# xiaomo9/FAC_fake

Measured on AMD Instinct MI355X. Metric: face-crops/sec at 224x224 bf16, CViT forward, 1/2/4/8 MI355X, higher is better.
Workload: dtype bf16; 1 GPU; config 2: CViT forward, B=256 crops per GPU per step, pos slot j mod 32; model=CViT(224,7,2,512,1024,6,8,2048), global_batch=256, seq_len=2, parallelism=frame-sharded x1, graph=False, stem_chunk=0, fused_stem224=True, pipelined=True

## Files before the change

fac_fake_amd/_lib.py:

```python
from __future__ import annotations

import ctypes
import os
from pathlib import Path

import torch

LIB_PATH = Path(os.environ.get("FAC_CVIT_LIB", Path(__file__).resolve().parent / "libfac_cvit.so"))

FAC_OK = 0
STATUS = {0: "FAC_OK", -1: "FAC_ERR_ARG", -2: "FAC_ERR_SHAPE", -3: "FAC_ERR_MISSING", -4: "FAC_ERR_HIP",
          -5: "FAC_ERR_NOT_LOADED", -6: "FAC_ERR_OOM"}
DTYPES = {"bf16": 0, "fp16": 1}

SIGNATURES = {
    "fac_create": (ctypes.c_int, [ctypes.c_int, ctypes.c_int, ctypes.POINTER(ctypes.c_void_p)]),
    "fac_load_weights": (ctypes.c_int, [ctypes.c_void_p, ctypes.c_void_p, ctypes.c_int]),
    "fac_reserve": (ctypes.c_int, [ctypes.c_void_p, ctypes.c_int]),
    "fac_workspace_bytes": (ctypes.c_int, [ctypes.c_void_p, ctypes.c_int, ctypes.POINTER(ctypes.c_size_t)]),
    "fac_forward_nchw_f32": (ctypes.c_int, [ctypes.c_void_p, ctypes.c_void_p, ctypes.c_int, ctypes.c_void_p,
                                            ctypes.c_void_p, ctypes.c_void_p, ctypes.c_void_p]),
    "fac_forward_nhwc_u8": (ctypes.c_int, [ctypes.c_void_p, ctypes.c_void_p, ctypes.c_int, ctypes.c_void_p,
                                           ctypes.c_void_p, ctypes.c_void_p, ctypes.c_void_p]),
    "fac_forward_nhwc_u8_pipelined": (ctypes.c_int, [ctypes.c_void_p, ctypes.c_void_p, ctypes.c_int,
# ... 66 lines not shown
                                             ctypes.c_int, ctypes.c_void_p]),
    "fac_s3d_base0_u8": (ctypes.c_int, [ctypes.c_void_p, ctypes.c_void_p, ctypes.c_void_p, ctypes.c_int, ctypes.c_int,
                                        ctypes.c_int, ctypes.c_void_p]),
    "fac_conv_nd_dual": (ctypes.c_int, [ctypes.c_void_p, ctypes.c_void_p, ctypes.c_void_p]),
    "fac_sep_tiny": (ctypes.c_int, [ctypes.c_void_p, ctypes.c_void_p, ctypes.c_void_p]),
    "fac_sep_mid": (ctypes.c_int, [ctypes.c_void_p, ctypes.c_void_p, ctypes.c_void_p]),
    "fac_bottleneck_pw2": (ctypes.c_int, [ctypes.c_void_p, ctypes.c_void_p, ctypes.c_void_p]),
    "fac_conv_weight_layout": (ctypes.c_int, [ctypes.c_int, ctypes.c_int, ctypes.c_int, ctypes.c_int, ctypes.c_int,
                                              ctypes.POINTER(ctypes.c_int), ctypes.POINTER(ctypes.c_int)]),
    "fac_pool_nd": (ctypes.c_int, [ctypes.c_void_p, ctypes.c_void_p]),
    "fac_pack_input": (ctypes.c_int, [ctypes.c_int, ctypes.c_void_p, ctypes.c_int, ctypes.c_int, ctypes.c_int,
                                      ctypes.c_float, ctypes.c_void_p, ctypes.c_void_p, ctypes.c_void_p, ctypes.c_int,
                                      ctypes.c_void_p]),
    "fac_pack_input_s2d": (ctypes.c_int, [ctypes.c_int, ctypes.c_void_p, ctypes.c_int, ctypes.c_int, ctypes.c_int,
                                          ctypes.c_int, ctypes.c_int, ctypes.c_int, ctypes.c_int, ctypes.c_float,
                                          ctypes.c_void_p, ctypes.c_void_p, ctypes.c_void_p, ctypes.c_void_p]),
    "fac_kan_linear": (ctypes.c_int, [ctypes.c_void_p, ctypes.c_int, ctypes.c_int, ctypes.c_int, ctypes.c_void_p,
                                      ctypes.c_int, ctypes.c_void_p, ctypes.c_void_p, ctypes.c_void_p,
                                      ctypes.c_void_p]),
    "fac_kan_scratch_bytes": (ctypes.c_size_t, [ctypes.c_int, ctypes.c_int, ctypes.c_int]),
    "fac_sigmoid": (ctypes.c_int, [ctypes.c_void_p, ctypes.c_void_p, ctypes.c_int, ctypes.c_void_p]),
    "fac_conv_nd_split": (ctypes.c_int, [ctypes.c_void_p, ctypes.c_void_p, ctypes.c_int, ctypes.c_int, ctypes.c_void_p,
                                          ctypes.c_int, ctypes.c_int, ctypes.c_void_p]),
    "fac_conv_nd_route": (ctypes.c_char_p, [ctypes.c_void_p, ctypes.c_int, ctypes.c_int,
                                            ctypes.POINTER(ctypes.c_int)]),
    "fac_conv_nd_dual_route": (ctypes.c_char_p, [ctypes.c_void_p, ctypes.c_void_p, ctypes.POINTER(ctypes.c_int)]),
    "fac_pool_nd_route": (ctypes.c_char_p, [ctypes.c_void_p, ctypes.POINTER(ctypes.c_int)]),
    "fac_conv3x3_packed_elems": (ctypes.c_size_t, [ctypes.c_int, ctypes.c_int, ctypes.c_int]),
    "fac_conv3x3_pack": (ctypes.c_int, [ctypes.c_int, ctypes.c_int, ctypes.c_int, ctypes.c_int, ctypes.c_void_p,
                                        ctypes.c_void_p]),
    "fac_conv3x3": (ctypes.c_int, [ctypes.c_int, ctypes.c_void_p, ctypes.c_void_p, ctypes.c_void_p, ctypes.c_void_p,
                                   ctypes.c_int, ctypes.c_int, ctypes.c_int, ctypes.c_int, ctypes.c_int, ctypes.c_int,
                                   ctypes.c_void_p, ctypes.c_void_p]),
    "fac_conv3x3_res_packed_elems": (ctypes.c_size_t, [ctypes.c_int, ctypes.c_int]),
    "fac_conv3x3_res_pack": (ctypes.c_int, [ctypes.c_int, ctypes.c_int, ctypes.c_int, ctypes.c_void_p,
                                            ctypes.c_void_p]),
    "fac_conv3x3_res": (ctypes.c_int, [ctypes.c_int, ctypes.c_void_p, ctypes.c_void_p, ctypes.c_void_p,
                                       ctypes.c_void_p, ctypes.c_void_p, ctypes.c_int, ctypes.c_int, ctypes.c_int,
                                       ctypes.c_void_p]),
    "fac_avgpool_f32": (ctypes.c_int, [ctypes.c_int, ctypes.c_void_p, ctypes.c_int, ctypes.c_int, ctypes.c_int,
                                       ctypes.c_void_p, ctypes.c_void_p]),
    "fac_stem224_pack_conv1": (ctypes.c_int, [ctypes.c_int, ctypes.c_void_p, ctypes.c_void_p]),
    "fac_stem224": (ctypes.c_int, [ctypes.c_int, ctypes.c_int, ctypes.c_void_p, ctypes.c_void_p, ctypes.c_void_p,
                                   ctypes.c_void_p, ctypes.c_void_p, ctypes.c_void_p, ctypes.c_void_p, ctypes.c_void_p,
                                   ctypes.c_int, ctypes.c_void_p]),
    "fac_ggca": (ctypes.c_int, [ctypes.c_int, ctypes.c_void_p, ctypes.c_int, ctypes.c_int, ctypes.c_int, ctypes.c_int,
                                ctypes.c_int, ctypes.c_void_p, ctypes.c_void_p, ctypes.c_void_p, ctypes.c_void_p,
                                ctypes.c_void_p, ctypes.c_void_p, ctypes.c_void_p]),
    "fac_ggca_apply_route": (ctypes.c_int, [ctypes.c_int, ctypes.c_int, ctypes.c_int, ctypes.c_int]),
    "fac_ggca_apply": (ctypes.c_int, [ctypes.c_int, ctypes.c_void_p, ctypes.c_int, ctypes.c_int, ctypes.c_int,
                                      ctypes.c_int, ctypes.c_int, ctypes.c_void_p, ctypes.c_void_p, ctypes.c_void_p,
                                      ctypes.c_void_p, ctypes.c_void_p, ctypes.c_int, ctypes.c_void_p,
                                      ctypes.c_void_p]),
    "fac_ggca_scale": (ctypes.c_int, [ctypes.c_int, ctypes.c_void_p, ctypes.c_int, ctypes.c_int, ctypes.c_int,
                                      ctypes.c_int, ctypes.c_int, ctypes.c_void_p, ctypes.c_void_p, ctypes.c_void_p,
                                      ctypes.c_void_p, ctypes.c_void_p, ctypes.c_void_p, ctypes.c_void_p]),
    "fac_idwconv": (ctypes.c_int, [ctypes.c_int, ctypes.c_void_p, ctypes.c_void_p, ctypes.c_int, ctypes.c_int,
                                   ctypes.c_int, ctypes.c_int, ctypes.c_void_p, ctypes.c_void_p, ctypes.c_void_p,
                                   ctypes.c_void_p, ctypes.c_void_p, ctypes.c_int, ctypes.c_void_p]),
    "fac_smfa_scratch_bytes": (ctypes.c_size_t, [ctypes.c_int, ctypes.c_int, ctypes.c_int, ctypes.c_int]),
    "fac_smfa_packed_bytes": (ctypes.c_size_t, [ctypes.c_int]),
    "fac_smfa_pack": (ctypes.c_int, [ctypes.c_int, ctypes.c_int] + [ctypes.c_void_p] * 12),
    "fac_smfa": (ctypes.c_int, [ctypes.c_int, ctypes.c_void_p, ctypes.c_int, ctypes.c_int, ctypes.c_int, ctypes.c_int,
                                ctypes.c_void_p, ctypes.c_int, ctypes.c_void_p, ctypes.c_void_p, ctypes.c_void_p,
                                ctypes.c_void_p]),
    "fac_bfm_packed_elems": (ctypes.c_size_t, [ctypes.c_int]),
# ... 97 lines not shown
```

fac_fake_amd/csrc/conv.hip:

```cpp
#include <cstdlib>
#include <type_traits>

#include "common.hpp"

namespace fac {

constexpr int CONV_CK = 32;

__device__ __forceinline__ void glds16(const void* gsrc, void* ldst) {
  __builtin_amdgcn_global_load_lds((const __attribute__((address_space(1))) void*)gsrc,
                                   (__attribute__((address_space(3))) void*)ldst, 16, 0, 0);
}

template <int TW>
constexpr int halo_rp() { return TW + 2 <= 24 ? 24 : 40; }

template <int TH, int TW, int BN>
constexpr int tile_res() {
  return TW == 16 ? (BN == 32 ? 224 : 112) : (TH == 8 ? 56 : (TH == 4 ? 28 : (TH == 14 ? 14 : 0)));
}

template <int TW>
__device__ __forceinline__ void box_pixel(int m, int& py, int& px) {
  constexpr int WW = TW / 2;
// ... 277 lines not shown
      if (c == 0) CONV_STAMP(2 + t);
#endif
    };
    step(std::integral_constant<int, 0>{});
    step(std::integral_constant<int, 1>{});
    step(std::integral_constant<int, 2>{});
    step(std::integral_constant<int, 3>{});
    step(std::integral_constant<int, 4>{});
    step(std::integral_constant<int, 5>{});
    step(std::integral_constant<int, 6>{});
    step(std::integral_constant<int, 7>{});
    step(std::integral_constant<int, 8>{});
  }
  asm volatile("s_waitcnt vmcnt(0)" ::: "memory");
  CONV_STAMP(11);
  const int Ho = POOL ? H / 2 : H, Wo = POOL ? W / 2 : W;
  const int oy0 = POOL ? y0 / 2 : y0, ox0 = POOL ? x0 / 2 : x0;
  __syncthreads();

  uint16_t* ostg = smem;
  if (do_relu)
    stage_tile<T, RTW, CTW, OPS, POOL, true>(acc, ostg, bias + nb * BN, wm, wn, lane);
  else
    stage_tile<T, RTW, CTW, OPS, POOL, false>(acc, ostg, bias + nb * BN, wm, wn, lane);
  __syncthreads();
  CONV_STAMP(12);
  store_tile<TH, TW, BN, POOL>(ostg, out, b, Ho, Wo, oy0, ox0, Cout, nb * BN, tid);
#ifdef CONV_STAMPS
  asm volatile("s_waitcnt vmcnt(0)" ::: "memory");
  CONV_STAMP(13);
#endif
}

template <class T, int TH, int TW, int BN, int WM, int WN, bool POOL, int OCC = 2, int BR = 3>
__global__ __launch_bounds__(256, OCC) void conv3x3_db(const uint16_t* __restrict__ in,
                                                       const uint16_t* __restrict__ wpk,
                                                       const float* __restrict__ bias, uint16_t* __restrict__ out,
                                                       int H, int W, int Cin, int Cout,
                                                       const uint16_t* __restrict__ zero16, int do_relu) {
  constexpr int CK = CONV_CK;
  constexpr int HH = TH + 2, HWD = TW + 2;
  constexpr int NPIX = TH * TW;
  constexpr int RT = ((NPIX + 15) / 16 + WM - 1) / WM * WM;
  constexpr int RTW = RT / WM;
  constexpr int CTW = BN / 16 / WN;
  constexpr int RPX = TW == 14 ? HWD + 1 : HWD;
  constexpr int HSLOTS = (HH * RPX * 4 + 255) / 256 * 256;
  constexpr int HPW = HSLOTS / 256;
  constexpr int HALO = HSLOTS * 8;
  constexpr int WSL = BN * CK;
  constexpr int OPS = BN + 8;
  constexpr int OPER = 2 * HALO;
  constexpr int OSTG = (POOL ? RT * 4 : RT * 16) * OPS;
  constexpr int SMEM = OPER > OSTG ? OPER : OSTG;
  static_assert(WM * WN == 4, "4 waves");
  static_assert(TH % 2 == 0 && TW % 2 == 0, "window-major order needs even boxes");
  static_assert(CTW * 16 * WN == BN, "BN split");
  __shared__ __attribute__((aligned(16))) uint16_t smem[SMEM];

  static_assert(tile_res<TH, TW, BN>() > 0, "tile shape without a resolution");
  H = W = tile_res<TH, TW, BN>();
  const int tid = threadIdx.x, lane = tid & 63, wave = tid >> 6;
  const int wm = wave / WN, wn = wave - (wave / WN) * WN;
  const int tiles_x = W / TW, tiles_per_img = (H / TH) * tiles_x;
  int bx = blockIdx.x;
  if ((gridDim.x & 7) == 0) bx = (bx & 7) * (gridDim.x >> 3) + (bx >> 3);
  const int b = bx / tiles_per_img;
  const int tile = bx - b * tiles_per_img;
  const int ty = tile / tiles_x, tx = tile - ty * tiles_x;
  const int y0 = ty * TH, x0 = tx * TW;
  const int nb = blockIdx.y;
  const int nchunks = Cin / CK;
  const int nsteps = nchunks * 9;
  const uint16_t* in_b = in + (size_t)b * H * W * Cin;
  const uint16_t* wsrc = wpk + (size_t)nb * nchunks * 9 * WSL;

  int hsrc[HPW];
#pragma unroll
  for (int i = 0; i < HPW; ++i) {
    const int slot = (i * 4 + wave) * 64 + lane;
    const int pix = slot >> 2;
    const int hy = pix / RPX, hx = pix - (pix / RPX) * RPX;
    const int q = hy < HH ? (slot & 3) ^ ((hy & 1) << 1) : 4;
    const int y = y0 + hy - 1, x = x0 + hx - 1;
    hsrc[i] = -1;
    if (q < 4 && hx < HWD && y >= 0 && y < H && x >= 0 && x < W) hsrc[i] = (y * W + x) * Cin + q * 8;
  }
  u16x8 hreg[HPW];
  auto load_halo = [&](int c) {
#pragma unroll
    for (int i = 0; i < HPW; ++i) {
      const uint16_t* src = hsrc[i] >= 0 ? in_b + hsrc[i] + c * CK : zero16;
      hreg[i] = *(const u16x8*)src;
    }
  };
  auto store_halo = [&](uint16_t* dst) {
#pragma unroll
    for (int i = 0; i < HPW; ++i) *(u16x8*)(dst + ((i * 4 + wave) * 64 + lane) * 8) = hreg[i];
  };
  const int boff = ((lane >> 4) * BN + wn * CTW * 16 + (lane & 15)) * 8;
  auto load_b = [&](u16x8(&dst)[CTW], int s) {
    const uint16_t* sb = wsrc + (size_t)(s < nsteps ? s : 0) * WSL + boff;
#pragma unroll
    for (int ct = 0; ct < CTW; ++ct) dst[ct] = *(const u16x8*)(sb + ct * 128);
  };

  int abase[RTW];
#pragma unroll
  for (int rt = 0; rt < RTW; ++rt) {
    int m = (wm * RTW + rt) * 16 + (lane & 15);
    if (m >= NPIX) m = 0;
    int py, px;
    box_pixel<TW>(m, py, px);
    abase[rt] = ((py * RPX + px) * 4 + ((lane >> 4) ^ ((py & 1) << 1))) * 8;
  }

  f32x4 acc[RTW][CTW];
#pragma unroll
  for (int rt = 0; rt < RTW; ++rt)
#pragma unroll
    for (int ct = 0; ct < CTW; ++ct) acc[rt][ct] = (f32x4)0.f;

  static_assert(BR == 3 || BR == 9, "B ring: 3 or 9 slices");
  u16x8 bq[BR][CTW];
  load_halo(0);
#pragma unroll
  for (int k = 0; k < BR - 1; ++k) load_b(bq[k], k);
  store_halo(smem);
  __syncthreads();
  u16x8 fa[RTW];
#pragma unroll
  for (int rt = 0; rt < RTW; ++rt) fa[rt] = *(const u16x8*)(smem + abase[rt]);

  for (int c = 0; c < nchunks; ++c) {
    const uint16_t* hb = smem + (c & 1) * HALO;
    uint16_t* hbn = smem + ((c + 1) & 1) * HALO;
    const int s0 = c * 9;
    auto step = [&](auto tc) {
      constexpr int t = decltype(tc)::value;
      load_b(bq[(t + BR - 1) % BR], s0 + t + BR - 1);
      if constexpr (t == 0) load_halo(c + 1 < nchunks ? c + 1 : c);
      constexpr int kyn = t < 8 ? (t + 1) / 3 : 0, kxn = t < 8 ? (t + 1) % 3 : 0;
      constexpr int ntoff = (kyn * RPX + kxn) * 32;
      const uint16_t* hnx = t < 8 ? hb : hbn;
#pragma unroll
      for (int rt = 0; rt < RTW; ++rt) {
#pragma unroll
        for (int ct = 0; ct < CTW; ++ct) acc[rt][ct] = T::mfma(fa[rt], bq[t % BR][ct], acc[rt][ct]);
        fa[rt] = *(const u16x8*)(hnx + abase[rt] + ntoff);
      }
      __builtin_amdgcn_sched_group_barrier(0x020, CTW + (t == 0 ? HPW : 0), 0);
#pragma unroll
      for (int rt = 0; rt < RTW; ++rt) {
        __builtin_amdgcn_sched_group_barrier(0x008, CTW, 0);
        __builtin_amdgcn_sched_group_barrier(0x100, 1, 0);
      }
      if constexpr (t == 1) store_halo(hbn);
      if constexpr (t == 7) asm volatile("s_waitcnt lgkmcnt(0)\n\ts_barrier" ::: "memory");
      __builtin_amdgcn_sched_barrier(0);
    };
    step(std::integral_constant<int, 0>{});
    step(std::integral_constant<int, 1>{});
    step(std::integral_constant<int, 2>{});
    step(std::integral_constant<int, 3>{});
    step(std::integral_constant<int, 4>{});
    step(std::integral_constant<int, 5>{});
    step(std::integral_constant<int, 6>{});
    step(std::integral_constant<int, 7>{});
    step(std::integral_constant<int, 8>{});
  }
  __syncthreads();

  uint16_t* ostg = smem;
  if (do_relu)
    stage_tile<T, RTW, CTW, OPS, POOL, true>(acc, ostg, bias + nb * BN, wm, wn, lane);
  else
    stage_tile<T, RTW, CTW, OPS, POOL, false>(acc, ostg, bias + nb * BN, wm, wn, lane);
  __syncthreads();
  const int Ho = POOL ? H / 2 : H, Wo = POOL ? W / 2 : W;
  const int oy0 = POOL ? y0 / 2 : y0, ox0 = POOL ? x0 / 2 : x0;
  store_tile<TH, TW, BN, POOL>(ostg, out, b, Ho, Wo, oy0, ox0, Cout, nb * BN, tid);
}

constexpr float kMean[3] = {0.485f, 0.456f, 0.406f};
constexpr float kStd[3] = {0.229f, 0.224f, 0.225f};

template <class T, bool U8>
__global__ __launch_bounds__(256) void conv1_bn_relu(const void* __restrict__ in_,
                                                     const uint16_t* __restrict__ w1,
                                                     const float* __restrict__ bias,
                                                     uint16_t* __restrict__ out, int H, int W) {
// ... 89 lines not shown
namespace fac {

int conv_block_n(int H, int cout) {
  switch (H) {
    case 224: return cout == 32 ? 32 : 0;
    case 112: return cout % 64 == 0 ? 64 : 0;
    case 56: return cout % 128 == 0 ? 128 : (cout % 64 == 0 ? 64 : 0);
    case 28:
      return cout % 256 == 0 ? 256 : (cout % 192 == 0 ? 192 : (cout % 128 == 0 ? 128 : 0));
    case 14: return cout % 128 == 0 ? 128 : (cout % 192 == 0 ? 192 : (cout % 64 == 0 ? 64 : 0));
    default: return 0;
  }
}

template <class T, int TH, int TW, int BN, int WM, int WN, int HB = 2, int OCC = 2, bool PB = true, bool POOLED = true,
          int WR = 3>
static hipError_t launch_box(const uint16_t* in, const uint16_t* wpk, const float* bias, uint16_t* out, int B, int H,
                             int Cin, int Cout, bool pool, const uint16_t* zero16, hipStream_t st, int relu) {
  dim3 grid(B * (H / TH) * (H / TW), Cout / BN);
  if constexpr (POOLED) {
    if (pool) {
      conv3x3_bn_relu<T, TH, TW, BN, WM, WN, true, HB, OCC, PB, WR>
          <<<grid, 256, 0, st>>>(in, wpk, bias, out, H, H, Cin, Cout, zero16, relu);
      return hipSuccess;
    }
  } else if (pool) {
    return hipErrorInvalidValue;
  }
  conv3x3_bn_relu<T, TH, TW, BN, WM, WN, false, HB, OCC, PB, WR>
      <<<grid, 256, 0, st>>>(in, wpk, bias, out, H, H, Cin, Cout, zero16, relu);
  return hipSuccess;
}

template <class T, int TH, int TW, int BN, int WM, int WN, int OCC = 2, int BR = 3>
static hipError_t launch_db(const uint16_t* in, const uint16_t* wpk, const float* bias, uint16_t* out, int B, int H,
                            int Cin, int Cout, bool pool, const uint16_t* zero16, hipStream_t st, int relu) {
  dim3 grid(B * (H / TH) * (H / TW), Cout / BN);
  if (pool)
    conv3x3_db<T, TH, TW, BN, WM, WN, true, OCC, BR>
        <<<grid, 256, 0, st>>>(in, wpk, bias, out, H, H, Cin, Cout, zero16, relu);
  else
    conv3x3_db<T, TH, TW, BN, WM, WN, false, OCC, BR>
        <<<grid, 256, 0, st>>>(in, wpk, bias, out, H, H, Cin, Cout, zero16, relu);
  return hipSuccess;
}



static int g_ring9 = 6;
void set_conv_ring9(int v) { g_ring9 = v; }
static int cu_count() {
  static int cached[64] = {0};
  int dev = 0;
  if (hipGetDevice(&dev) != hipSuccess || dev < 0 || dev >= 64) return 256;
  if (!cached[dev]) {
    int n = 0;
    cached[dev] = hipDeviceGetAttribute(&n, hipDeviceAttributeMultiprocessorCount, dev) == hipSuccess && n > 0 ? n : 256;
  }
  return cached[dev];
}

template <class T>
static hipError_t launch_conv_t(const uint16_t* in, const uint16_t* wpk, const float* bias, uint16_t* out,
                                int B, int H, int W, int Cin, int Cout, bool pool, const uint16_t* z, hipStream_t st,
                                int relu, int bn) {
  if (W != H) return hipErrorInvalidValue;
  if (bn == 0) bn = conv_block_n(H, Cout);
  if (bn <= 0 || Cout % bn) return hipErrorInvalidValue;
  const bool few = g_ring9 && (long)B * (Cout / bn) * (H == 14 ? 1 : H == 28 ? 7 : 1 << 30) <= 2L * cu_count();
  const int ring9 = few ? g_ring9 : 0;
  switch (H * 1000 + bn) {
    case 224032: launch_box<T, 16, 16, 32, 4, 1, 2, 2, false>(in, wpk, bias, out, B, H, Cin, Cout, pool, z, st, relu); break;
    case 112064:
      if (pool)
        launch_box<T, 16, 16, 64, 4, 1, 1, 2, false>(in, wpk, bias, out, B, H, Cin, Cout, pool, z, st, relu);
      else
        launch_box<T, 16, 16, 64, 4, 1, 1, 4, false>(in, wpk, bias, out, B, H, Cin, Cout, pool, z, st, relu);
      break;
    case 56128: launch_box<T, 8, 28, 128, 2, 2>(in, wpk, bias, out, B, H, Cin, Cout, pool, z, st, relu); break;
    case 56064: launch_box<T, 8, 28, 64, 2, 2>(in, wpk, bias, out, B, H, Cin, Cout, pool, z, st, relu); break;
    case 28256: launch_db<T, 4, 28, 256, 1, 4>(in, wpk, bias, out, B, H, Cin, Cout, pool, z, st, relu); break;
    case 28192: launch_db<T, 4, 28, 192, 1, 4>(in, wpk, bias, out, B, H, Cin, Cout, pool, z, st, relu); break;
    case 28128:
      if (ring9 & 4)
        launch_db<T, 4, 28, 128, 1, 4, 2, 9>(in, wpk, bias, out, B, H, Cin, Cout, pool, z, st, relu);
      else
        launch_db<T, 4, 28, 128, 1, 4>(in, wpk, bias, out, B, H, Cin, Cout, pool, z, st, relu);
      break;
    case 14128:
      launch_box<T, 14, 14, 128, 1, 4, 2, 2, false>(in, wpk, bias, out, B, H, Cin, Cout, pool, z, st, relu);
      break;
    case 14192:
      if (launch_box<T, 14, 14, 192, 1, 4, 2, 2, false, false>(in, wpk, bias, out, B, H, Cin, Cout, pool, z, st, relu) != hipSuccess)
        return hipErrorInvalidValue;
      break;
    case 14032:
      if (ring9 & 2)
        launch_box<T, 14, 14, 32, 4, 1, 2, 2, true, true, 9>(in, wpk, bias, out, B, H, Cin, Cout, pool, z, st, relu);
      else
        launch_box<T, 14, 14, 32, 4, 1, 2, 2, true>(in, wpk, bias, out, B, H, Cin, Cout, pool, z, st, relu);
      break;
    case 14064:
      if (ring9 & 2)
        launch_box<T, 14, 14, 64, 1, 4, 2, 2, true, true, 9>(in, wpk, bias, out, B, H, Cin, Cout, pool, z, st, relu);
      else if (ring9 & 1)
        launch_box<T, 14, 14, 64, 1, 4, 2, 2, false, true, 9>(in, wpk, bias, out, B, H, Cin, Cout, pool, z, st, relu);
      else
        launch_box<T, 14, 14, 64, 1, 4, 2, 2, false>(in, wpk, bias, out, B, H, Cin, Cout, pool, z, st, relu);
      break;
    default: return hipErrorInvalidValue;
  }
  return hipGetLastError();
// ... 24 lines not shown
```

fac_fake_amd/csrc/cvit_abi.hip:

```cpp
#include <hip/hip_runtime.h>

#include <algorithm>
#include <atomic>
#include <cmath>
#include <cstdio>
#include <cstring>
#include <map>
#include <string>
#include <vector>

#include "../../include/fac_cvit.h"
#include "common.hpp"
#include "ops_common.hpp"

namespace fac {
void set_conv_ring9(int v);
int conv_block_n(int H, int cout);
void set_gemm_small(int max_m, int variant);
void pack_conv3x3(int dtype, int H, int ci, int co, const float* w, uint16_t* out, int bn = 0);
void pack_stem_conv1(int dtype, const float* w, uint16_t* out);
hipError_t launch_conv3x3(int dtype, const uint16_t* in, const uint16_t* wpk, const float* bias, uint16_t* out,
                          int B, int H, int W, int Cin, int Cout, bool pool, const uint16_t* zero16, hipStream_t st, bool relu = true,
                          int bn = 0);
hipError_t launch_conv1(int dtype, bool u8, const void* in, const uint16_t* w1, const float* bias, uint16_t* out,
                        int B, int H, int W, hipStream_t st);
hipError_t launch_gemm(int dtype, int epi, const uint16_t* A, int lda, const uint16_t* W, int ldw, const float* bias,
                       void* out, int ldo, int M, int N, int K, int splits, hipStream_t st, int variant = -1);
hipError_t launch_embed_finalize_ln(int dtype, const float* slab, int S, int B, const float* bias, const float* cls,
                                    const float* pos, const int32_t* pidx, float* x, const float* g, const float* bt,
                                    uint16_t* y, int* err, int seq, hipStream_t st);
hipError_t launch_resid_layernorm(int dtype, float* x, const float* slab, int S, const float* bias, const float* g,
                                 const float* b, uint16_t* y, int R, hipStream_t st, float eps = 1e-5f);
hipError_t launch_resid_cls(int dtype, const float* x, const float* slab, int S, const float* bias, uint16_t* c, int B,
                            hipStream_t st);
hipError_t launch_attention2(int dtype, const float* qkv, uint16_t* o, int B, float scale, hipStream_t st);
hipError_t launch_head_out(const float* hid, const float* w2, const float* b2, float* logits, float* probs, int B,
                           hipStream_t st);
hipError_t launch_video_score(const float* logits, int n, float* score, hipStream_t st);
hipError_t launch_video_score_seg(const float* logits, const int* seg, int nv, float* score, hipStream_t st);
hipError_t launch_crop_resize(const uint8_t* frames, int n_frames, int H, int W, const int32_t* boxes, int n_boxes,
                              uint8_t* crops, hipStream_t st);
hipError_t launch_clip_stage(const uint8_t* frames, int n_frames, int H, int W, const int32_t* boxes, int n_boxes,
                             int T, uint8_t* clips, hipStream_t st);
hipError_t launch_stem224(int dtype, bool u8, const void* in, const uint16_t* w1, const float* b1, const uint16_t* w2,
                          const float* b2, const uint16_t* w3, const float* b3, uint16_t* out, int B, int nwg,
                          hipStream_t s);
size_t dgrad_partial_floats(int M, int N, int K);
hipError_t launch_dgrad(int dtype, const float* dY, int ldy, const uint16_t* W, float* P, int M, int N, int K,
                        int* splits, hipStream_t st);
// ... 872 lines not shown
}

int fac_reserve(fac_ctx* c, int max_batch) {
  if (!c || max_batch <= 0) return set_err(c, FAC_ERR_ARG, "bad reserve arguments");
  DevGuard g(c->device);
  return ensure_ws(c, max_batch);
}

int fac_workspace_bytes(fac_ctx* c, int B, size_t* out) {
  if (!c || !out || B <= 0) return FAC_ERR_ARG;
  *out = layout(B, c->stem_chunk).total;
  return FAC_OK;
}

int fac_set_stem_chunk(fac_ctx* c, int crops) {
  if (!c || crops < 0) return FAC_ERR_ARG;
  if (crops != c->stem_chunk) {
    DevGuard g(c->device);
    drop_graphs(c);
    c->stem_chunk = crops;
    const int cap = c->cap_B;
    c->cap_B = 0;
    if (cap > 0) {
      DevGuard g(c->device);
      return ensure_ws(c, cap);
    }
  }
  return FAC_OK;
}

int fac_set_option(fac_ctx* c, const char* key, int value) {
  if (!c || !key) return FAC_ERR_ARG;
  const std::string k(key);
  {
    DevGuard g(c->device);
    drop_graphs(c);
    c->knob_gen = ++g_knob_gen;
  }
  if (k == "stem_chunk") return fac_set_stem_chunk(c, value);
  if (k == "conv_ring9") {
    if (value < 0 || value > 7) return set_err(c, FAC_ERR_ARG, "conv_ring9 must be 0..7");
    fac::set_conv_ring9(value);
    return FAC_OK;
  }
  if (k == "conv_small14") {
    c->small14 = value != 0;
    return FAC_OK;
  }
  if (k == "conv_small") {
    c->conv_small = value != 0;
    return FAC_OK;
  }
  if (k == "graph_max_b") {
    if (value < 0 || value > 256) return set_err(c, FAC_ERR_ARG, "graph_max_b must be 0..256");
    c->graph_max_b = value;
    return FAC_OK;
  }
  if (k == "tail_only") {
    if (c->loaded) return set_err(c, FAC_ERR_ARG, "tail_only must be set before fac_load_weights");
    c->tail_only = value != 0;
    return FAC_OK;
  }
  if (k == "fuse_stem224") {
    c->fuse_stem224 = value != 0;
    return FAC_OK;
  }
  if (k == "stem_events") {
    c->stem_ev = value != 0;
    c->stem_ev_used = 0;
    return FAC_OK;
  }
  if (k == "nd_occ3") {
    if (value < 0) return set_err(c, FAC_ERR_ARG, "nd_occ3 must be >= 0");
    fac::set_nd_occ3(value);
    return FAC_OK;
  }
  if (k == "nd_pt_wide") {
// ... 408 lines not shown
```

fac_fake_amd/csrc/stack_ops.hip:

```cpp
#include <hip/hip_runtime.h>

#include <vector>

#include "../../include/fac_cvit.h"
#include "../../include/fac_ops.h"
#include "common.hpp"

namespace fac {

int conv_block_n(int H, int cout);
hipError_t launch_conv3x3(int dtype, const uint16_t* in, const uint16_t* wpk, const float* bias, uint16_t* out,
                          int B, int H, int W, int Cin, int Cout, bool pool, const uint16_t* zero16, hipStream_t st,
                          bool relu, int bn = 0);
hipError_t launch_stem224(int dtype, bool u8, const void* in, const uint16_t* w1, const float* b1, const uint16_t* w2,
                          const float* b2, const uint16_t* w3, const float* b3, uint16_t* out, int B, int nwg,
                          hipStream_t s);

static inline uint16_t to16(int dtype, float f) {
  return dtype == 0 ? fac_host::f32_to_bf16(f) : fac_host::f32_to_f16(f);
}

void pack_conv3x3(int dtype, int H, int ci, int co, const float* w, uint16_t* out, int bn) {
  const int BN = bn ? bn : conv_block_n(H, co), CK = 32, nch = ci / CK;
  size_t q = 0;
  for (int nb = 0; nb < co / BN; ++nb)
    for (int ch = 0; ch < nch; ++ch)
      for (int t = 0; t < 9; ++t)
        for (int qq = 0; qq < CK / 8; ++qq) {
          const int qs = (H != 224 && (t / 3) % 2 == 1) ? qq ^ 2 : qq;
          for (int nl = 0; nl < BN; ++nl)
            for (int j = 0; j < 8; ++j)
              out[q++] = to16(dtype, w[((size_t)(nb * BN + nl) * ci + ch * CK + qs * 8 + j) * 9 + t]);
        }
}

void pack_stem_conv1(int dtype, const float* w, uint16_t* out) {
  for (int i = 0; i < 32 * 64; ++i) out[i] = 0;
  for (int o = 0; o < 32; ++o)
    for (int t = 0; t < 9; ++t)
      for (int cin = 0; cin < 3; ++cin) {
        const int ky = t / 3, kx = t % 3;
        out[(size_t)o * 64 + ((ky * 2 + kx / 2) * 2 + kx % 2) * 4 + cin] = to16(dtype, w[((size_t)o * 3 + cin) * 9 + t]);
      }
// ... 2 lines not shown
static bool conv3x3_shape_ok(int h, int cin, int cout) {
  if (h != 224 && h != 112 && h != 56 && h != 28 && h != 14) return false;
  if (cin < 32 || cin % 32 || cout <= 0) return false;
  return conv_block_n(h, cout) > 0;
}

static int num_cus() {
  static int cached[64] = {0};
  int dev = 0;
  if (hipGetDevice(&dev) != hipSuccess || dev < 0 || dev >= 64) return 256;
  if (!cached[dev]) {
    int n = 0;
    if (hipDeviceGetAttribute(&n, hipDeviceAttributeMultiprocessorCount, dev) != hipSuccess || n <= 0) n = 256;
    cached[dev] = n;
  }
  return cached[dev];
}

}

extern "C" {

size_t fac_conv3x3_packed_elems(int h, int cin, int cout) {
  return fac::conv3x3_shape_ok(h, cin, cout) ? (size_t)cout * cin * 9 : 0;
}

int fac_conv3x3_pack(int dtype, int h, int cin, int cout, const float* w, uint16_t* out) {
  if (!w || !out || (dtype != 0 && dtype != 1)) return FAC_ERR_ARG;
  if (!fac::conv3x3_shape_ok(h, cin, cout)) return FAC_ERR_SHAPE;
  fac::pack_conv3x3(dtype, h, cin, cout, w, out, 0);
  return FAC_OK;
}

int fac_conv3x3(int dtype, const void* in, const void* wpk, const float* bias, void* out, int n, int h, int cin,
                int cout, int pool, int relu, const void* zero256, void* stream) {
  if (!in || !wpk || !bias || !out || !zero256 || n <= 0 || (dtype != 0 && dtype != 1)) return FAC_ERR_ARG;
  if (!fac::conv3x3_shape_ok(h, cin, cout)) return FAC_ERR_SHAPE;
  if (pool && h == 14 && fac::conv_block_n(h, cout) == 192) return FAC_ERR_SHAPE;
  const hipError_t e = fac::launch_conv3x3(dtype, (const uint16_t*)in, (const uint16_t*)wpk, bias, (uint16_t*)out, n,
                                           h, h, cin, cout, pool != 0, (const uint16_t*)zero256,
                                           (hipStream_t)stream, relu != 0);
  return e == hipSuccess ? FAC_OK : FAC_ERR_HIP;
}

int fac_stem224_pack_conv1(int dtype, const float* w, uint16_t* out) {
  if (!w || !out || (dtype != 0 && dtype != 1)) return FAC_ERR_ARG;
  fac::pack_stem_conv1(dtype, w, out);
  return FAC_OK;
}

int fac_stem224(int dtype, int u8, const void* in, const void* w1p, const float* b1, const void* w2, const float* b2,
                const void* w3, const float* b3, void* out, int n, void* stream) {
  if (!in || !w1p || !b1 || !w2 || !b2 || !w3 || !b3 || !out || n <= 0 || (dtype != 0 && dtype != 1))
    return FAC_ERR_ARG;
  const hipError_t e = fac::launch_stem224(dtype, u8 != 0, in, (const uint16_t*)w1p, b1, (const uint16_t*)w2, b2,
                                           (const uint16_t*)w3, b3, (uint16_t*)out, n, fac::num_cus(),
                                           (hipStream_t)stream);
  return e == hipSuccess ? FAC_OK : FAC_ERR_HIP;
}

}
```

include/fac_ops.h:

```cpp
#ifndef FAC_OPS_H
#define FAC_OPS_H

#include <stddef.h>
#include <stdint.h>

#ifdef __cplusplus
extern "C" {
#endif

#define FAC_CONV_RELU 1
#define FAC_CONV_RESID 2
#define FAC_CONV_RELU2 4
#define FAC_CONV_OUT_F32 8
#define FAC_CONV_MAXPOOL3S2 16
#define FAC_CONV_PREPOOL3S2 64
#define FAC_CONV_MAXPOOL3S1 32

typedef struct fac_conv_desc {
  int dtype;
  const void* in;
  int n, d, h, w, cin;
  const void* weight;
  const float* bias;
  int cout, k_pad;
// ... 81 lines not shown
typedef struct {
  int dtype;
  const void* in;
  int ldi, i_off;
  int n, t, h, w, c;
  int kt, k;
  const float* ws;
  const float* wt;
  const float* scale;
  const float* shift;
  int act;
  const float* scale2;
  const float* shift2;
  void* out;
  int ldo, o_off;
  int out_f32;
} fac_dwsep_desc;
int fac_dwsep3d(const fac_dwsep_desc* desc, void* stream);

int fac_bn_maxpool3d(int dtype, const void* in, int ldi, int i_off, int n, int t, int h, int w, int c, int kt,
                     const float* scale, const float* shift, void* out, int ldo, int o_off, void* stream);

#define FAC_EW_AFFINE 0
#define FAC_EW_GELU 1
#define FAC_EW_MUL 2
#define FAC_EW_ADD 3
#define FAC_EW_ADD_GELU 4
#define FAC_EW_CLAMP6 5
#define FAC_EW_ADD3 6
int fac_ew(int dtype, int op, const void* a, int lda, int a_off, const void* b, int ldb, int b_off, const void* c3,
           int ldc, int c_off, const float* scale, const float* shift, void* out, int ldo, int o_off, long long rows,
           int c, void* stream);

size_t fac_conv3x3_packed_elems(int h, int cin, int cout);
int fac_conv3x3_pack(int dtype, int h, int cin, int cout, const float* w, uint16_t* out);
int fac_conv3x3(int dtype, const void* in, const void* wpk, const float* bias, void* out, int n, int h, int cin,
                int cout, int pool, int relu, const void* zero256, void* stream);

int fac_stem224_pack_conv1(int dtype, const float* w, uint16_t* out);
int fac_stem224(int dtype, int u8, const void* in, const void* w1p, const float* b1, const void* w2, const float* b2,
                const void* w3, const float* b3, void* out, int n, void* stream);

size_t fac_conv3x3_res_packed_elems(int h, int c);
int fac_conv3x3_res_pack(int dtype, int h, int c, const float* w, uint16_t* out);
int fac_conv3x3_res(int dtype, const void* in, const void* wpk, const float* bias, const void* residual, void* out,
                    int n, int h, int c, void* stream);

int fac_avgpool_f32(int dtype, const void* x, int n, int s, int c, float* y, void* stream);

int fac_idwconv(int dtype, const void* in, void* out, int n, int h, int w, int c, const float* w_hw, const float* w_w,
                const float* w_h, const float* scale, const float* shift, int pool, void* stream);

size_t fac_smfa_scratch_bytes(int n, int h, int w, int c);
size_t fac_smfa_packed_bytes(int c);
int fac_smfa_pack(int dtype, int c, const float* w0, const float* b0, const float* gate4, const float* w1,
                  const float* b1, const float* dww, const float* dwb, const float* wpw, const float* bpw,
                  const float* wcat, const float* bcat, void* out);
int fac_smfa(int dtype, const void* x, int n, int h, int w, int c, const void* wpk, int residual, void* out,
             float* gate_out, void* scratch, void* stream);

size_t fac_bfm_packed_elems(int c);
int fac_bfm_pack(int dtype, int c, const float* w3, const float* w5, const float* w7, uint16_t* out);
int fac_bfm(int dtype, const void* x, int n, int h, int w, int c, const void* wpk, const float* bias3, float scale,
            void* out, void* stream);

int fac_sigmoid(const float* x, float* y, int n, void* stream);
// ... 7 lines not shown
```

Measured before the change: 85450 face-crops/s.

## Add persistent wave-per-box 3x3 conv kernel for 112x112 layers

Adds a persistent kernel for 112x112 3x3 convs with 64 output channels. It keeps all weights in LDS for the whole launch and gives each of 12 waves its own 8x8 output box, with a private halo buffer and no block-level syncs in the main loop. The kernel is used by default once the batch yields enough boxes, and option knobs can force it on or off or cap the grid. The aim is to cut repeated weight reloads and block synchronisation in the existing box kernel. The cost is a single-occupancy, LDS-heavy launch and serialised load-then-compute per wave, with little latency hiding.

```diff
diff --git a/fac_fake_amd/_lib.py b/fac_fake_amd/_lib.py
--- a/fac_fake_amd/_lib.py
+++ b/fac_fake_amd/_lib.py
@@ -122,6 +122,7 @@
     "fac_conv3x3": (ctypes.c_int, [ctypes.c_int, ctypes.c_void_p, ctypes.c_void_p, ctypes.c_void_p, ctypes.c_void_p,
                                    ctypes.c_int, ctypes.c_int, ctypes.c_int, ctypes.c_int, ctypes.c_int, ctypes.c_int,
                                    ctypes.c_void_p, ctypes.c_void_p]),
+    "fac_conv112_wave_min_boxes": (ctypes.c_int, []),
     "fac_conv3x3_res_packed_elems": (ctypes.c_size_t, [ctypes.c_int, ctypes.c_int]),
     "fac_conv3x3_res_pack": (ctypes.c_int, [ctypes.c_int, ctypes.c_int, ctypes.c_int, ctypes.c_void_p,
                                             ctypes.c_void_p]),
diff --git a/fac_fake_amd/csrc/conv.hip b/fac_fake_amd/csrc/conv.hip
--- a/fac_fake_amd/csrc/conv.hip
+++ b/fac_fake_amd/csrc/conv.hip
@@ -333,6 +333,186 @@
 #endif
 }
 
+template <class T, int NCH, bool POOL, int NW>
+__global__ __launch_bounds__(NW * 64, 1) void conv3x3_wave(const uint16_t* __restrict__ in,
+                                                          const uint16_t* __restrict__ wpk,
+                                                          const float* __restrict__ bias,
+                                                          uint16_t* __restrict__ out, int nboxes,
+                                                          const uint16_t* __restrict__ zero16, int do_relu) {
+  constexpr int CK = CONV_CK, H = 112, W = 112, Cin = NCH * CK, Cout = 64;
+  constexpr int TB = 8, HB = TB + 2;
+  constexpr int HSLOTS = HB * HB * 4;
+  constexpr int HI = (HSLOTS + 63) / 64;
+  constexpr int HALO = HI * 64 * 8;
+  constexpr int WSL = 64 * CK;
+  constexpr int WEL = NCH * 9 * WSL;
+  constexpr int OPS = 64 + 8;
+  constexpr int TPI = (H / TB) * (W / TB);
+  static_assert((POOL ? 16 : 32) * OPS <= HALO, "epilogue tile in the halo buffer");
+  __shared__ __attribute__((aligned(16))) uint16_t smem[WEL + NW * HALO + 128];
+
+  const int tid = threadIdx.x, lane = tid & 63;
+  const int wave = __builtin_amdgcn_readfirstlane(tid >> 6);
+  for (int p = tid; p < WEL / 8; p += NW * 64) ((u16x8*)smem)[p] = ((const u16x8*)wpk)[p];
+  const float* const sbias = (const float*)(smem + WEL + NW * HALO);
+  if (tid < 64) ((float*)(smem + WEL + NW * HALO))[tid] = bias[tid];
+  __syncthreads();
+
+  uint16_t* const hbuf = smem + WEL + wave * HALO;
+  int hmap[HI];
+#pragma unroll
+  for (int i = 0; i < HI; ++i) {
+    const int slot = i * 64 + lane, pix = slot >> 2;
+    const int hy = pix / HB, hx = pix - hy * HB;
+    const int q = (slot & 3) ^ ((hy & 1) << 1);
+    const int edge = slot >= HSLOTS ? 16 : (hy == 0) | (hy == HB - 1) << 1 | (hx == 0) << 2 | (hx == HB - 1) << 3;
+    hmap[i] = (((hy - 1) * W + (hx - 1)) * (Cin / 8) + q) * 32 | edge;
+  }
+  int abase[4], bbase[4];
+#pragma unroll
+  for (int rt = 0; rt < 4; ++rt) {
+    int py, px;
+    box_pixel<TB>(rt * 16 + (lane & 15), py, px);
+    abase[rt] = ((py * HB + px) * 4 + ((lane >> 4) ^ ((py & 1) << 1))) * 8;
+  }
+#pragma unroll
+  for (int ct = 0; ct < 4; ++ct) bbase[ct] = ((lane >> 4) * 64 + ct * 16 + (lane & 15)) * 8;
+
+  int v = blockIdx.x;
+  const int G = gridDim.x;
+  if ((G & 7) == 0) v = (v & 7) * (G >> 3) + (v >> 3);
+  for (int box = v * NW + wave; box < nboxes; box += G * NW) {
+    const int b = box / TPI, tile = box - b * TPI;
+    const int ty = tile / (W / TB), tx = tile - ty * (W / TB);
+    const int y0 = ty * TB, x0 = tx * TB;
+    const uint16_t* const in_o = in + (size_t)b * H * W * Cin + (y0 * W + x0) * Cin;
+    const int emask = 16 | (y0 == 0) | (y0 == H - TB) << 1 | (x0 == 0) << 2 | (x0 == W - TB) << 3;
+
+    f32x4 acc[4][4];
+#pragma unroll
+    for (int rt = 0; rt < 4; ++rt)
+#pragma unroll
+      for (int ct = 0; ct < 4; ++ct) acc[rt][ct] = (f32x4)0.f;
+
+#pragma unroll
+    for (int c = 0; c < NCH; ++c) {
+      asm volatile("s_waitcnt lgkmcnt(0)" ::: "memory");
+      __builtin_amdgcn_sched_barrier(0);
+#pragma unroll
+      for (int i = 0; i < HI; ++i) {
+        int hm;
+        asm volatile("v_mov_b32 %0, %1" : "=v"(hm) : "v"(hmap[i]));
+        const uint16_t* src = (hm & emask) ? zero16 : in_o + (hm >> 5) * 8 + c * CK;
+        glds16(src, hbuf + i * 64 * 8);
+      }
+      asm volatile("s_waitcnt vmcnt(0)" ::: "memory");
+      __builtin_amdgcn_sched_barrier(0);
+      const uint16_t* const wb = smem + c * 9 * WSL;
+      u16x8 fa[4], bcur[4];
+#pragma unroll
+      for (int ct = 0; ct < 4; ++ct) bcur[ct] = *(const u16x8*)(wb + bbase[ct]);
+#pragma unroll
+      for (int rt = 0; rt < 4; ++rt) fa[rt] = *(const u16x8*)(hbuf + abase[rt]);
+      __builtin_amdgcn_sched_barrier(0);
+#pragma unroll
+      for (int t = 0; t < 9; ++t) {
+        const int kyn = (t + 1) / 3, kxn = (t + 1) % 3;
+        const int ntoff = (kyn * HB + kxn) * 32;
+        u16x8 bfr[4], bnx[4];
+#pragma unroll
+        for (int ct = 0; ct < 4; ++ct) bfr[ct] = bcur[ct];
+#pragma unroll
+        for (int rt = 0; rt < 4; ++rt) {
+#pragma unroll
+          for (int ct = 0; ct < 4; ++ct) acc[rt][ct] = T::mfma(fa[rt], bfr[ct], acc[rt][ct]);
+          if (t < 8) {
+            fa[rt] = *(const u16x8*)(hbuf + abase[rt] + ntoff);
+            if (rt == 0) {
+#pragma unroll
+              for (int ct = 0; ct < 4; ++ct) bnx[ct] = *(const u16x8*)(wb + (t + 1) * WSL + bbase[ct]);
+            }
+          }
+        }
+        if (t < 8) {
+#pragma unroll
+          for (int ct = 0; ct < 4; ++ct) bcur[ct] = bnx[ct];
+          __builtin_amdgcn_sched_group_barrier(0x008, 4, 0);
+          __builtin_amdgcn_sched_group_barrier(0x100, 5, 0);
+#pragma unroll
+          for (int rt = 1; rt < 4; ++rt) {
+            __builtin_amdgcn_sched_group_barrier(0x008, 4, 0);
+            __builtin_amdgcn_sched_group_barrier(0x100, 1, 0);
+          }
+        }
+        __builtin_amdgcn_sched_barrier(0);
+      }
+    }
+
+    asm volatile("s_waitcnt lgkmcnt(0)" ::: "memory");
+    __builtin_amdgcn_sched_barrier(0);
+    auto epilogue = [&](auto rl) {
+      constexpr bool RELU = decltype(rl)::value;
+      float bv[4];
+#pragma unroll
+      for (int ct = 0; ct < 4; ++ct) bv[ct] = sbias[ct * 16 + (lane & 15)];
+      if constexpr (POOL) {
+  #pragma unroll
+        for (int ct = 0; ct < 4; ++ct)
+  #pragma unroll
+          for (int rt = 0; rt < 4; ++rt) {
+            const f32x4 a = acc[rt][ct];
+            const float mx = fmaxf(fmaxf(a[0], a[1]), fmaxf(a[2], a[3])) + bv[ct];
+            hbuf[(rt * 4 + (lane >> 4)) * OPS + ct * 16 + (lane & 15)] = T::from_f32(RELU ? relu(mx) : mx);
+          }
+        __builtin_amdgcn_wave_barrier();
+        asm volatile("" ::: "memory");
+        uint16_t* const ob = out + ((size_t)b * (H / 2) * (W / 2) + (y0 / 2) * (W / 2) + x0 / 2) * Cout;
+  #pragma unroll
+        for (int k = 0; k < 2; ++k) {
+          const int it = k * 64 + lane, w = it >> 3, q = it & 7;
+          const u16x8 val = *(const u16x8*)(hbuf + w * OPS + q * 8);
+          *(u16x8*)(ob + ((w >> 2) * (W / 2) + (w & 3)) * Cout + q * 8) = val;
+        }
+      } else {
+        uint16_t* const ob = out + ((size_t)b * H * W + y0 * W + x0) * Cout;
+  #pragma unroll
+        for (int h = 0; h < 2; ++h) {
+  #pragma unroll
+          for (int ct = 0; ct < 4; ++ct)
+  #pragma unroll
+            for (int r2 = 0; r2 < 2; ++r2) {
+              const f32x4 a = acc[2 * h + r2][ct];
+              f32x4 y;
+  #pragma unroll
+              for (int j = 0; j < 4; ++j) y[j] = RELU ? relu(a[j] + bv[ct]) : a[j] + bv[ct];
+              const uint32_t p01 = T::pack2(y[0], y[1]), p23 = T::pack2(y[2], y[3]);
+              uint16_t* const o = hbuf + (r2 * 16 + (lane >> 4) * 4) * OPS + ct * 16 + (lane & 15);
+              o[0] = (uint16_t)p01;
+              o[OPS] = (uint16_t)(p01 >> 16);
+              o[2 * OPS] = (uint16_t)p23;
+              o[3 * OPS] = (uint16_t)(p23 >> 16);
+            }
+          __builtin_amdgcn_wave_barrier();
+          asm volatile("" ::: "memory");
+  #pragma unroll
+          for (int k = 0; k < 4; ++k) {
+            const int ly = (lane >> 4) & 1, lx = 2 * (lane >> 5) + ((lane >> 3) & 1);
+            const unsigned loff = (ly * W + lx) * Cout + (lane & 7) * 8;
+            const u16x8 val = *(const u16x8*)(hbuf + (k * 8 + (lane >> 3)) * OPS + (lane & 7) * 8);
+            *(u16x8*)(ob + ((4 * h + 2 * (k >> 1)) * W + 4 * (k & 1)) * Cout + loff) = val;
+          }
+          __builtin_amdgcn_wave_barrier();
+          asm volatile("" ::: "memory");
+        }
+      }
+    };
+    if (do_relu)
+      epilogue(std::true_type{});
+    else
+      epilogue(std::false_type{});
+  }
+}
+
 template <class T, int TH, int TW, int BN, int WM, int WN, bool POOL, int OCC = 2, int BR = 3>
 __global__ __launch_bounds__(256, OCC) void conv3x3_db(const uint16_t* __restrict__ in,
                                                        const uint16_t* __restrict__ wpk,
@@ -641,6 +821,38 @@
   return cached[dev];
 }
 
+constexpr int WAVE112_NW = 12;
+constexpr int WAVE112_MIN_BOXES = 8 * 256 * WAVE112_NW;
+static int g_wave112 = 1, g_wave112_nwg = 0;
+bool set_conv112_wave(int v) {
+  if (v < 0 || v > 2) return false;
+  g_wave112 = v;
+  return true;
+}
+bool set_conv112_wave_nwg(int v) {
+  if (v < 0) return false;
+  g_wave112_nwg = v;
+  return true;
+}
+int conv112_wave_min_boxes() { return WAVE112_MIN_BOXES; }
+
+template <class T>
+static void launch_wave(const uint16_t* in, const uint16_t* wpk, const float* bias, uint16_t* out, int B, int Cin,
+                        bool pool, const uint16_t* z, hipStream_t st, int relu) {
+  constexpr int NW = WAVE112_NW;
+  const int nboxes = B * 196;
+  int grid = (nboxes + NW - 1) / NW;
+  if (grid > cu_count()) grid = cu_count();
+  if (g_wave112_nwg > 0 && grid > g_wave112_nwg) grid = g_wave112_nwg;
+  if (Cin == 32) {
+    if (pool) conv3x3_wave<T, 1, true, NW><<<grid, NW * 64, 0, st>>>(in, wpk, bias, out, nboxes, z, relu);
+    else conv3x3_wave<T, 1, false, NW><<<grid, NW * 64, 0, st>>>(in, wpk, bias, out, nboxes, z, relu);
+  } else {
+    if (pool) conv3x3_wave<T, 2, true, NW><<<grid, NW * 64, 0, st>>>(in, wpk, bias, out, nboxes, z, relu);
+    else conv3x3_wave<T, 2, false, NW><<<grid, NW * 64, 0, st>>>(in, wpk, bias, out, nboxes, z, relu);
+  }
+}
+
 template <class T>
 static hipError_t launch_conv_t(const uint16_t* in, const uint16_t* wpk, const float* bias, uint16_t* out,
                                 int B, int H, int W, int Cin, int Cout, bool pool, const uint16_t* z, hipStream_t st,
@@ -653,7 +865,10 @@
   switch (H * 1000 + bn) {
     case 224032: launch_box<T, 16, 16, 32, 4, 1, 2, 2, false>(in, wpk, bias, out, B, H, Cin, Cout, pool, z, st, relu); break;
     case 112064:
-      if (pool)
+      if (Cout == 64 && (Cin == 32 || Cin == 64) && B < (1 << 23) &&
+          (g_wave112 == 2 || (g_wave112 == 1 && (long)B * 196 >= WAVE112_MIN_BOXES)))
+        launch_wave<T>(in, wpk, bias, out, B, Cin, pool, z, st, relu);
+      else if (pool)
         launch_box<T, 16, 16, 64, 4, 1, 1, 2, false>(in, wpk, bias, out, B, H, Cin, Cout, pool, z, st, relu);
       else
         launch_box<T, 16, 16, 64, 4, 1, 1, 4, false>(in, wpk, bias, out, B, H, Cin, Cout, pool, z, st, relu);
diff --git a/fac_fake_amd/csrc/cvit_abi.hip b/fac_fake_amd/csrc/cvit_abi.hip
--- a/fac_fake_amd/csrc/cvit_abi.hip
+++ b/fac_fake_amd/csrc/cvit_abi.hip
@@ -15,6 +15,8 @@
 
 namespace fac {
 void set_conv_ring9(int v);
+bool set_conv112_wave(int v);
+bool set_conv112_wave_nwg(int v);
 int conv_block_n(int H, int cout);
 void set_gemm_small(int max_m, int variant);
 void pack_conv3x3(int dtype, int H, int ci, int co, const float* w, uint16_t* out, int bn = 0);
@@ -953,6 +955,14 @@
 int fac_set_option(fac_ctx* c, const char* key, int value) {
   if (!c || !key) return FAC_ERR_ARG;
   const std::string k(key);
+  if (k == "conv112_wave" || k == "conv112_wave_nwg") {
+    if (!(k == "conv112_wave" ? fac::set_conv112_wave(value) : fac::set_conv112_wave_nwg(value)))
+      return set_err(c, FAC_ERR_ARG, k == "conv112_wave" ? "conv112_wave must be 0, 1 or 2" : "conv112_wave_nwg must be >= 0");
+    DevGuard g(c->device);
+    drop_graphs(c);
+    c->knob_gen = ++g_knob_gen;
+    return FAC_OK;
+  }
   {
     DevGuard g(c->device);
     drop_graphs(c);
diff --git a/fac_fake_amd/csrc/stack_ops.hip b/fac_fake_amd/csrc/stack_ops.hip
--- a/fac_fake_amd/csrc/stack_ops.hip
+++ b/fac_fake_amd/csrc/stack_ops.hip
@@ -9,6 +9,7 @@
 namespace fac {
 
 int conv_block_n(int H, int cout);
+int conv112_wave_min_boxes();
 hipError_t launch_conv3x3(int dtype, const uint16_t* in, const uint16_t* wpk, const float* bias, uint16_t* out,
                           int B, int H, int W, int Cin, int Cout, bool pool, const uint16_t* zero16, hipStream_t st,
                           bool relu, int bn = 0);
@@ -77,6 +78,8 @@
   return FAC_OK;
 }
 
+int fac_conv112_wave_min_boxes(void) { return fac::conv112_wave_min_boxes(); }
+
 int fac_conv3x3(int dtype, const void* in, const void* wpk, const float* bias, void* out, int n, int h, int cin,
                 int cout, int pool, int relu, const void* zero256, void* stream) {
   if (!in || !wpk || !bias || !out || !zero256 || n <= 0 || (dtype != 0 && dtype != 1)) return FAC_ERR_ARG;
diff --git a/include/fac_ops.h b/include/fac_ops.h
--- a/include/fac_ops.h
+++ b/include/fac_ops.h
@@ -137,6 +137,7 @@
            int ldc, int c_off, const float* scale, const float* shift, void* out, int ldo, int o_off, long long rows,
            int c, void* stream);
 
+int fac_conv112_wave_min_boxes(void);
 size_t fac_conv3x3_packed_elems(int h, int cin, int cout);
 int fac_conv3x3_pack(int dtype, int h, int cin, int cout, const float* w, uint16_t* out);
 int fac_conv3x3(int dtype, const void* in, const void* wpk, const float* bias, void* out, int n, int h, int cin,
```

Result: no change. 86200 face-crops/s (median of 6 runs) (+0.9%).

## Route 56x56 Cout-128 conv to double-buffered kernel with reduced A-fragment ring

Applied to the files above, without the earlier changes.

Adds an A-operand register ring depth (AD) to the double-buffered 3x3 conv kernel. Fewer fragment registers are kept live, and the next tap's fragments are prefetched across row tiles, with the chunk barrier moved into the last tap. Address bases are computed for only a periodic subset of row tiles, with the rest reached through a constant shift. The 56x56, 128-channel conv now uses this kernel with a 1x4 wave layout and an A-ring depth of 3 instead of the box kernel, behind a new option that is on by default. The aim is to cut register pressure and improve MFMA/LDS overlap, at the risk of different tile efficiency and a changed barrier placement.

```diff
diff --git a/fac_fake_amd/csrc/conv.hip b/fac_fake_amd/csrc/conv.hip
--- a/fac_fake_amd/csrc/conv.hip
+++ b/fac_fake_amd/csrc/conv.hip
@@ -333,7 +333,7 @@
 #endif
 }
 
-template <class T, int TH, int TW, int BN, int WM, int WN, bool POOL, int OCC = 2, int BR = 3>
+template <class T, int TH, int TW, int BN, int WM, int WN, bool POOL, int OCC = 2, int BR = 3, int AD_ = 0>
 __global__ __launch_bounds__(256, OCC) void conv3x3_db(const uint16_t* __restrict__ in,
                                                        const uint16_t* __restrict__ wpk,
                                                        const float* __restrict__ bias, uint16_t* __restrict__ out,
@@ -354,9 +354,11 @@
   constexpr int OPER = 2 * HALO;
   constexpr int OSTG = (POOL ? RT * 4 : RT * 16) * OPS;
   constexpr int SMEM = OPER > OSTG ? OPER : OSTG;
+  constexpr int AD = AD_ > 0 ? AD_ : RTW;
   static_assert(WM * WN == 4, "4 waves");
   static_assert(TH % 2 == 0 && TW % 2 == 0, "window-major order needs even boxes");
   static_assert(CTW * 16 * WN == BN, "BN split");
+  static_assert(AD <= RTW && (9 * RTW) % AD == 0, "A ring: a position's slot must not depend on the chunk");
   __shared__ __attribute__((aligned(16))) uint16_t smem[SMEM];
 
   static_assert(tile_res<TH, TW, BN>() > 0, "tile shape without a resolution");
@@ -406,9 +408,13 @@
     for (int ct = 0; ct < CTW; ++ct) dst[ct] = *(const u16x8*)(sb + ct * 128);
   };
 
-  int abase[RTW];
-#pragma unroll
-  for (int rt = 0; rt < RTW; ++rt) {
+  constexpr int WW = TW / 2;
+  constexpr int AP0 = WW % 4 == 0 ? WW / 4 : (WW % 2 == 0 ? WW / 2 : WW);
+  constexpr int AP = (NPIX == RT * 16 && RTW % AP0 == 0) ? AP0 : RTW;
+  constexpr int ASH = (4 * AP / WW) * 2 * RPX * 32;
+  int abase[AP];
+#pragma unroll
+  for (int rt = 0; rt < AP; ++rt) {
     int m = (wm * RTW + rt) * 16 + (lane & 15);
     if (m >= NPIX) m = 0;
     int py, px;
@@ -429,35 +435,47 @@
   for (int k = 0; k < BR - 1; ++k) load_b(bq[k], k);
   store_halo(smem);
   __syncthreads();
-  u16x8 fa[RTW];
-#pragma unroll
-  for (int rt = 0; rt < RTW; ++rt) fa[rt] = *(const u16x8*)(smem + abase[rt]);
+  u16x8 fa[AD];
+#pragma unroll
+  for (int rt = 0; rt < AD; ++rt) fa[rt] = *(const u16x8*)(smem + abase[rt % AP] + (rt / AP) * ASH);
 
   for (int c = 0; c < nchunks; ++c) {
     const uint16_t* hb = smem + (c & 1) * HALO;
     uint16_t* hbn = smem + ((c + 1) & 1) * HALO;
     const int s0 = c * 9;
+    auto rows = [&](auto tc, auto r0c, auto r1c) {
+      constexpr int t = decltype(tc)::value, R0 = decltype(r0c)::value, R1 = decltype(r1c)::value;
+#pragma unroll
+      for (int rt = R0; rt < R1; ++rt) {
+#pragma unroll
+        for (int ct = 0; ct < CTW; ++ct) acc[rt][ct] = T::mfma(fa[(t * RTW + rt) % AD], bq[t % BR][ct], acc[rt][ct]);
+        const int tn = rt + AD < RTW ? t : t + 1, rn = rt + AD < RTW ? rt + AD : rt + AD - RTW;
+        const int kyn = tn < 9 ? tn / 3 : 0, kxn = tn < 9 ? tn % 3 : 0;
+        fa[(t * RTW + rt) % AD] =
+            *(const u16x8*)((tn < 9 ? hb : hbn) + abase[rn % AP] + (rn / AP) * ASH + (kyn * RPX + kxn) * 32);
+      }
+#pragma unroll
+      for (int rt = R0; rt < R1; ++rt) {
+        __builtin_amdgcn_sched_group_barrier(0x008, CTW, 0);
+        __builtin_amdgcn_sched_group_barrier(0x100, 1, 0);
+      }
+    };
+    using std::integral_constant;
     auto step = [&](auto tc) {
       constexpr int t = decltype(tc)::value;
       load_b(bq[(t + BR - 1) % BR], s0 + t + BR - 1);
       if constexpr (t == 0) load_halo(c + 1 < nchunks ? c + 1 : c);
-      constexpr int kyn = t < 8 ? (t + 1) / 3 : 0, kxn = t < 8 ? (t + 1) % 3 : 0;
-      constexpr int ntoff = (kyn * RPX + kxn) * 32;
-      const uint16_t* hnx = t < 8 ? hb : hbn;
-#pragma unroll
-      for (int rt = 0; rt < RTW; ++rt) {
-#pragma unroll
-        for (int ct = 0; ct < CTW; ++ct) acc[rt][ct] = T::mfma(fa[rt], bq[t % BR][ct], acc[rt][ct]);
-        fa[rt] = *(const u16x8*)(hnx + abase[rt] + ntoff);
-      }
       __builtin_amdgcn_sched_group_barrier(0x020, CTW + (t == 0 ? HPW : 0), 0);
-#pragma unroll
-      for (int rt = 0; rt < RTW; ++rt) {
-        __builtin_amdgcn_sched_group_barrier(0x008, CTW, 0);
-        __builtin_amdgcn_sched_group_barrier(0x100, 1, 0);
+      if constexpr (AD < RTW && t == 8) {
+        rows(tc, integral_constant<int, 0>{}, integral_constant<int, RTW - AD>{});
+        asm volatile("s_waitcnt lgkmcnt(0)\n\ts_barrier" ::: "memory");
+        __builtin_amdgcn_sched_barrier(0);
+        rows(tc, integral_constant<int, RTW - AD>{}, integral_constant<int, RTW>{});
+      } else {
+        rows(tc, integral_constant<int, 0>{}, integral_constant<int, RTW>{});
       }
       if constexpr (t == 1) store_halo(hbn);
-      if constexpr (t == 7) asm volatile("s_waitcnt lgkmcnt(0)\n\ts_barrier" ::: "memory");
+      if constexpr (AD == RTW && t == 7) asm volatile("s_waitcnt lgkmcnt(0)\n\ts_barrier" ::: "memory");
       __builtin_amdgcn_sched_barrier(0);
     };
     step(std::integral_constant<int, 0>{});
@@ -613,23 +631,25 @@
   return hipSuccess;
 }
 
-template <class T, int TH, int TW, int BN, int WM, int WN, int OCC = 2, int BR = 3>
+template <class T, int TH, int TW, int BN, int WM, int WN, int OCC = 2, int BR = 3, int AD = 0>
 static hipError_t launch_db(const uint16_t* in, const uint16_t* wpk, const float* bias, uint16_t* out, int B, int H,
                             int Cin, int Cout, bool pool, const uint16_t* zero16, hipStream_t st, int relu) {
   dim3 grid(B * (H / TH) * (H / TW), Cout / BN);
   if (pool)
-    conv3x3_db<T, TH, TW, BN, WM, WN, true, OCC, BR>
+    conv3x3_db<T, TH, TW, BN, WM, WN, true, OCC, BR, AD>
         <<<grid, 256, 0, st>>>(in, wpk, bias, out, H, H, Cin, Cout, zero16, relu);
   else
-    conv3x3_db<T, TH, TW, BN, WM, WN, false, OCC, BR>
+    conv3x3_db<T, TH, TW, BN, WM, WN, false, OCC, BR, AD>
         <<<grid, 256, 0, st>>>(in, wpk, bias, out, H, H, Cin, Cout, zero16, relu);
   return hipSuccess;
 }
 
 
-
 static int g_ring9 = 6;
 void set_conv_ring9(int v) { g_ring9 = v; }
+
+static int g_db_wide = 1;
+void set_conv_db_wide(int v) { g_db_wide = v; }
 static int cu_count() {
   static int cached[64] = {0};
   int dev = 0;
@@ -658,7 +678,12 @@
       else
         launch_box<T, 16, 16, 64, 4, 1, 1, 4, false>(in, wpk, bias, out, B, H, Cin, Cout, pool, z, st, relu);
       break;
-    case 56128: launch_box<T, 8, 28, 128, 2, 2>(in, wpk, bias, out, B, H, Cin, Cout, pool, z, st, relu); break;
+    case 56128:
+      if (g_db_wide)
+        launch_db<T, 8, 28, 128, 1, 4, 2, 3, 3>(in, wpk, bias, out, B, H, Cin, Cout, pool, z, st, relu);
+      else
+        launch_box<T, 8, 28, 128, 2, 2>(in, wpk, bias, out, B, H, Cin, Cout, pool, z, st, relu);
+      break;
     case 56064: launch_box<T, 8, 28, 64, 2, 2>(in, wpk, bias, out, B, H, Cin, Cout, pool, z, st, relu); break;
     case 28256: launch_db<T, 4, 28, 256, 1, 4>(in, wpk, bias, out, B, H, Cin, Cout, pool, z, st, relu); break;
     case 28192: launch_db<T, 4, 28, 192, 1, 4>(in, wpk, bias, out, B, H, Cin, Cout, pool, z, st, relu); break;
diff --git a/fac_fake_amd/csrc/cvit_abi.hip b/fac_fake_amd/csrc/cvit_abi.hip
--- a/fac_fake_amd/csrc/cvit_abi.hip
+++ b/fac_fake_amd/csrc/cvit_abi.hip
@@ -15,6 +15,7 @@
 
 namespace fac {
 void set_conv_ring9(int v);
+void set_conv_db_wide(int v);
 int conv_block_n(int H, int cout);
 void set_gemm_small(int max_m, int variant);
 void pack_conv3x3(int dtype, int H, int ci, int co, const float* w, uint16_t* out, int bn = 0);
@@ -964,6 +965,11 @@
     fac::set_conv_ring9(value);
     return FAC_OK;
   }
+  if (k == "conv_db_wide") {
+    if (value < 0 || value > 1) return set_err(c, FAC_ERR_ARG, "conv_db_wide must be 0 or 1");
+    fac::set_conv_db_wide(value);
+    return FAC_OK;
+  }
   if (k == "conv_small14") {
     c->small14 = value != 0;
     return FAC_OK;
```

Result: no change. 85320 face-crops/s before, 85370 face-crops/s after (median of 3 runs) (+0.1%).
